# CarbonMatrixLab/AbX

Hardware: AMD Instinct MI355X
Metric: diffusion-steps/sec (100 samples, ~350-res complex) (higher is better)
Workload: dtype f32; 1 GPU; L352: L=352 (Lab 228 + antigen 124), 100 samples of one complex over 1 GPU(s), 1 step = ScoreNetwork (3 passes) + get_prev + reverse, seeded random weights, ESM off; L=352, samples_total=100, chunk=auto, parallelism=sample-shard x1, no collective in the step

## Files before the change

### abx_amd/csrc/gemm_as.hip

```cpp
#include <stdlib.h>

#include <type_traits>

#include "common.h"
#include "abx_hip.h"

namespace {

typedef __attribute__((address_space(3))) void* lds_ptr_t;
typedef const __attribute__((address_space(1))) void* glb_ptr_t;

constexpr int AS_BM = 64, AS_BN = 128, AS_NK = 12, AS_RING = 3;
constexpr int AS_KT = 4096;
constexpr int AS_A = AS_NK * AS_KT;
constexpr int AS_STAGE = 2 * AS_BN * 32;
constexpr int AS_HALF = AS_KT / 2;
constexpr int AS_OFF_RING = AS_A;
constexpr int AS_OFF_ST = AS_OFF_RING + AS_RING * AS_STAGE;
constexpr int AS_OFF_CONST = AS_OFF_ST + 4 * 64 * 4;
constexpr int AS_LDS = AS_OFF_CONST + 2 * 1024;

__device__ __forceinline__ void as_glds16(const void* src, char* dst_wave_base) {
    __builtin_amdgcn_global_load_lds((glb_ptr_t)src, (lds_ptr_t)dst_wave_base, 16, 0, 0);
}
__device__ __forceinline__ unsigned as_vgpr32(unsigned o) {
    asm volatile("" : "+v"(o));
    return o;
}
template <int I> using IC = std::integral_constant<int, I>;
template <int I0, int I1, class F> __device__ __forceinline__ void as_static_for(F&& f) {
    if constexpr (I0 < I1) {
        f(IC<I0>{});
        as_static_for<I0 + 1, I1>(f);
    }
}

template <int ROWS> __device__ __forceinline__ int as_plane_off(int plane, int row, int half) {
    return plane * (ROWS * 32) + row * 32 + ((half ^ ((row >> 3) & 1)) << 4);
}

__device__ __forceinline__ long long as_a_row(const AbxGemm& g, int gri) {
    long long gr = gri;
    if (g.a_pair) {
        int pi, pj;
        if (g.c_split_tile) {
            pair_tile_decode(gri, g.pair_Lp, pi, pj);
            pi = min(pi, g.pair_L - 1);
            pj = min(pj, g.pair_L - 1);
        } else {
            pi = gri / g.pair_Lp;
            pj = min(gri - pi * g.pair_Lp, g.pair_L - 1);
        }
        gr = g.a_pair_transpose > 0 ? (long long)pj * g.pair_L + pi : (long long)pi * g.pair_L + pj;
    } else if (g.a_pair_transpose > 0) {
        const int qi = gri / g.a_pair_transpose;
        gr = (long long)(gri - qi * g.a_pair_transpose) * g.a_pair_transpose + qi;
    }
    return gr;
}

__device__ __forceinline__ void as_issue_a(const AbxGemm& g, char* lds, int m0, int b, int wm) {
    const int lane = threadIdx.x & 63;
    const bool remap = g.a_pair_transpose > 0 || g.a_pair != 0;
    const long long row0 = remap ? 0 : m0;
    const char* baseA = reinterpret_cast<const char*>(g.A + (long long)b * g.sAb + row0 * g.sAm);
    unsigned offA[2];
#pragma unroll
    for (int i = 0; i < 2; ++i) {
        const int r = 16 * i + (lane >> 2), p = lane & 3;
        const int kq = p ^ ((r >> 2) & 3);
        const long long gr = as_a_row(g, min(m0 + wm * 32 + r, g.M - 1));
        offA[i] = (unsigned)(((gr - row0) * g.sAm + kq * 4) * 4);
    }
    char* dst = lds + wm * AS_HALF;
#pragma unroll
    for (int kt = 0; kt < AS_NK; ++kt)
#pragma unroll
        for (int i = 0; i < 2; ++i) as_glds16(baseA + kt * 64 + as_vgpr32(offA[i]), dst + kt * AS_KT + i * 1024);
}

struct AsConv {
    float lshift, m2048;
    f32x2 ls2, lq2;
    int rd0, rd1, wr;
    bool ln, relu;
};
__device__ __forceinline__ void as_conv_init(AsConv& c, const AbxGemm& g) {
    const int lane = threadIdx.x & 63, r = lane & 31, h = lane >> 5, x = (r >> 2) & 3;
    c.rd0 = r * 64 + (((2 * h) ^ x) << 4);
    c.rd1 = r * 64 + (((2 * h + 1) ^ x) << 4);
    c.wr = as_plane_off<32>(0, r, h);
    c.lshift = 0.f;
    c.ls2 = c.lq2 = (f32x2){0.f, 0.f};
    c.m2048 = -2048.0f;
    asm volatile("" : "+v"(c.m2048));
    c.ln = g.ln_csum != nullptr;
    c.relu = g.a_relu != 0;
}
template <bool FIRST>
__device__ __forceinline__ void as_conv_ktile(AsConv& c, char* img) {
    const int lane = threadIdx.x & 63;
    const f32x4 lo = *reinterpret_cast<const f32x4*>(img + c.rd0);
    const f32x4 hi = *reinterpret_cast<const f32x4*>(img + c.rd1);
    float xv[8];
#pragma unroll
    for (int e = 0; e < 4; ++e) { xv[e] = lo[e]; xv[4 + e] = hi[e]; }
    if (c.ln) {
        if (FIRST) c.lshift = __shfl(xv[0], lane & 31, 64);
        const f32x2 sh2 = {c.lshift, c.lshift};
#pragma unroll
        for (int e = 0; e < 4; ++e) {
            f32x2 xp = {xv[2 * e], xv[2 * e + 1]};
            xp -= sh2;
            c.ls2 += xp;
            c.lq2 = __builtin_elementwise_fma(xp, xp, c.lq2);
            xv[2 * e] = xp[0];
            xv[2 * e + 1] = xp[1];
        }
    }
    if (c.relu) {
#pragma unroll
        for (int e = 0; e < 8; ++e) xv[e] = fmaxf(xv[e], 0.f);
    }
    unsigned q0[4], q1[4];
#pragma unroll
    for (int e = 0; e < 4; ++e) split2h_mix(xv[2 * e], xv[2 * e + 1], c.m2048, q0[e], q1[e]);
    *reinterpret_cast<u32x4*>(img + c.wr) = u32x4{q0[0], q0[1], q0[2], q0[3]};
    *reinterpret_cast<u32x4*>(img + c.wr + 1024) = u32x4{q1[0], q1[1], q1[2], q1[3]};
}
__device__ __forceinline__ void as_conv_finish(const AsConv& c, float* st, int wm, float eps, float cs) {
    const int lane = threadIdx.x & 63;
    const float ls = c.ls2[0] + c.ls2[1], lq = c.lq2[0] + c.lq2[1];
    const float invK = 1.0f / (float)(AS_NK * 16);
    const float sm = ls + __shfl_xor(ls, 32, 64), sq = lq + __shfl_xor(lq, 32, 64);
    if (lane < 32) {
        const float dm = sm * invK;
        st[wm * 32 + lane] = dm;
        st[64 + wm * 32 + lane] = (1.0f / sqrtf(fmaxf(sq * invK - dm * dm, 0.f) + eps)) * cs;
    }
}

__device__ __forceinline__ void as_quad_transpose(const float (&x)[4], float (&o)[4]) {
    float a0, a1, a2, a3;
    asm volatile(
        "s_nop 1\n\t"
        "s_mov_b32 vcc_lo, 0x55555555\n\ts_mov_b32 vcc_hi, 0x55555555\n\t"
        "v_cndmask_b32_dpp %4, %9, %8, vcc quad_perm:[1,0,3,2] row_mask:0xf bank_mask:0xf\n\t"
        "v_cndmask_b32_dpp %6, %11, %10, vcc quad_perm:[1,0,3,2] row_mask:0xf bank_mask:0xf\n\t"
        "s_mov_b32 vcc_lo, 0xaaaaaaaa\n\ts_mov_b32 vcc_hi, 0xaaaaaaaa\n\t"
        "v_cndmask_b32_dpp %5, %8, %9, vcc quad_perm:[1,0,3,2] row_mask:0xf bank_mask:0xf\n\t"
        "v_cndmask_b32_dpp %7, %10, %11, vcc quad_perm:[1,0,3,2] row_mask:0xf bank_mask:0xf\n\t"
        "s_mov_b32 vcc_lo, 0x33333333\n\ts_mov_b32 vcc_hi, 0x33333333\n\t"
        "v_cndmask_b32_dpp %0, %6, %4, vcc quad_perm:[2,3,0,1] row_mask:0xf bank_mask:0xf\n\t"
        "v_cndmask_b32_dpp %1, %7, %5, vcc quad_perm:[2,3,0,1] row_mask:0xf bank_mask:0xf\n\t"
        "s_mov_b32 vcc_lo, 0xcccccccc\n\ts_mov_b32 vcc_hi, 0xcccccccc\n\t"
        "v_cndmask_b32_dpp %2, %4, %6, vcc quad_perm:[2,3,0,1] row_mask:0xf bank_mask:0xf\n\t"
        "v_cndmask_b32_dpp %3, %5, %7, vcc quad_perm:[2,3,0,1] row_mask:0xf bank_mask:0xf"
        : "=&v"(o[0]), "=&v"(o[1]), "=&v"(o[2]), "=&v"(o[3]), "=&v"(a0), "=&v"(a1), "=&v"(a2), "=&v"(a3)
        : "v"(x[0]), "v"(x[1]), "v"(x[2]), "v"(x[3])
        : "vcc");
}

template <int S0, int NSL, int NST, int NDMA = 4>
struct AsSched {
    static_assert(S0 >= 2 && S0 + NSL <= 10, "slice window");
    static constexpr int after(int kt, bool first) { return (kt == 0 ? 2 : 0) + ((!first && kt >= S0 && kt < S0 + NSL) ? NST : 0); }
    static constexpr int allow(int kt, bool first) {
        const int k2 = (kt + AS_NK - 2) % AS_NK, k1 = (kt + AS_NK - 1) % AS_NK;
        return after(k2, first) + NDMA + after(k1, first);
    }
};

enum { AS_EPI_PLAIN = 0, AS_EPI_GLU = 1 };

template <int N>
__device__ __forceinline__ void as_rendezvous(u32x4 (&fa)[2], u32x4 (&fb)[2][2]) {
    asm volatile("s_waitcnt vmcnt(%6) lgkmcnt(0)\n\ts_barrier"
                 : "+v"(fa[0]), "+v"(fa[1]), "+v"(fb[0][0]), "+v"(fb[0][1]), "+v"(fb[1][0]), "+v"(fb[1][1])
                 : "n"(N)
                 : "memory");
}
__device__ __forceinline__ void as_rendezvous_free(u32x4 (&fa)[2], u32x4 (&fb)[2][2]) {
    asm volatile("s_waitcnt lgkmcnt(0)\n\ts_barrier"
                 : "+v"(fa[0]), "+v"(fa[1]), "+v"(fb[0][0]), "+v"(fb[0][1]), "+v"(fb[1][0]), "+v"(fb[1][1])
                 :
                 : "memory");
}
template <int N> __device__ __forceinline__ void as_wait_vm() { asm volatile("s_waitcnt vmcnt(%0)" ::"n"(N) : "memory"); }

template <int EPI, bool SIDE, bool EDGE, int ABL = 0, bool PL = false>
__device__ __forceinline__ void as_block(const AbxGemm& g, const AbxGemm& s2, char* lds, int mt, int b) {
    const int lane = threadIdx.x & 63, wave = __builtin_amdgcn_readfirstlane(threadIdx.x >> 6);
    const int wm = wave >> 1, wn = wave & 1, h = lane >> 5;
    const int m0 = mt * AS_BM;
    float* st = reinterpret_cast<float*>(lds + AS_OFF_ST);
    using Sched = typename std::conditional<EPI == AS_EPI_PLAIN, AsSched<2, 8, (ABL == 1 ? 0 : (PL ? 2 : 1)), (ABL == 3 ? 2 : 4)>, AsSched<6, 2, (ABL == 1 ? 0 : 2), (ABL == 3 ? 2 : 4)>>::type;

    const int ntiles = (g.N + AS_BN - 1) / AS_BN;
    const bool ragged = (g.N % AS_BN) != 0;
    const char* bbase = reinterpret_cast<const char*>(g.B_split);
    const long long bkstep = g.sB3k * 2;
    unsigned off0, offU[2];
    {
        const int row = lane >> 1, hp = lane & 1;
        off0 = (unsigned)((wm * g.sB3p + (long long)row * g.sB3n + 8 * (hp ^ ((row >> 3) & 1))) * 2);
#pragma unroll
        for (int i = 2; i < 4; ++i) {
            const int r2 = i * 32 + row;
            const int half = hp ^ ((row >> 3) & 1);
            if (SIDE) offU[i - 2] = (unsigned)((wm * s2.sB3p + (long long)min(r2 - 64, s2.N - 1) * s2.sB3n + 8 * half) * 2);
            else offU[i - 2] = (unsigned)((wm * g.sB3p + (long long)min((ntiles - 1) * AS_BN + r2, g.N - 1) * g.sB3n + 8 * half) * 2);
        }
    }
    const char* bbaseS = SIDE ? reinterpret_cast<const char*>(s2.B_split) : bbase;
    const long long bkstepS = SIDE ? s2.sB3k * 2 : bkstep;
    const unsigned tile_step = (unsigned)(AS_BN * g.sB3n * 2), chunk_step = (unsigned)(32 * g.sB3n * 2);
    auto issue_b = [&](int tile, int kt, int slot, bool half_only = false) __attribute__((always_inline)) {
        char* dst = lds + AS_OFF_RING + slot * AS_STAGE + wm * 4096;
        const int t = min(tile, ntiles - 1);
        const char* src = bbase + kt * bkstep + (long long)t * tile_step;
#pragma unroll
        for (int i = 0; i < 2; ++i) as_glds16(src + i * chunk_step + as_vgpr32(off0), dst + i * 1024);
        if (half_only) return;
        if (t == ntiles - 1) {
            const char* srcU = bbaseS + kt * bkstepS;
#pragma unroll
            for (int i = 2; i < 4; ++i) as_glds16(srcU + as_vgpr32(offU[i - 2]), dst + i * 1024);
        } else {
#pragma unroll
            for (int i = 2; i < 4; ++i) as_glds16(src + i * chunk_step + as_vgpr32(off0), dst + i * 1024);
        }
    };
    const float* csrc = (wm ? g.bias : g.ln_csum);
    auto issue_consts = [&](int tile) __attribute__((always_inline)) {
        const int t = min(tile, ntiles - 1);
#pragma unroll
        for (int i = 0; i < 2; ++i) {
            const int n = min(t * AS_BN + i * 64 + lane, g.N - 1);
            char* dst = lds + AS_OFF_CONST + (tile & 1) * 1024 + wm * 512 + i * 256;
            __builtin_amdgcn_global_load_lds((glb_ptr_t)(csrc + n), (lds_ptr_t)dst, 4, 0, 0);
        }
    };

#ifdef ABX_AS_STAMP
    unsigned long long t_wait = 0, t_vm = 0, t_bar = 0;
    const unsigned long long t_begin = __builtin_amdgcn_s_memtime();
    unsigned long long t_issued = 0, as_t_landed = 0;
#endif
    AsConv cv;
    char* a_half = lds + wm * AS_HALF;
    if (wn == 0) {
        as_issue_a(g, lds, m0, b, wm);
#ifdef ABX_AS_STAMP
        t_issued = __builtin_amdgcn_s_memtime();
#endif
        as_conv_init(cv, g);
        as_wait_vm<20>();
#ifdef ABX_AS_STAMP
        as_t_landed = __builtin_amdgcn_s_memtime();
#endif
        as_conv_ktile<true>(cv, a_half);
        as_conv_ktile<false>(cv, a_half + AS_KT);
    } else {
        issue_b(0, 0, 0);
        issue_b(0, 1, 1);
        issue_b(0, 2, 2);
        if (EPI == AS_EPI_GLU && wm == 0) {
            const int m = m0 + lane;
            int pi, pj;
            pair_tile_decode(m, g.pair_Lp, pi, pj);
            const bool ok = m < g.M && pi < g.pair_L && pj < g.c_split_L;
            st[128 + lane] = (ok && g.rowscale) ? g.rowscale[(long long)b * g.sRSb + (long long)pi * g.pair_Lp + pj] : (ok ? 1.f : 0.f);
            st[192 + lane] = ok ? 1.f : 0.f;
        }
        as_wait_vm<8>();
    }
    __syncthreads();

    const float cs = __builtin_ldexpf(1.0f, -ABX_F16_A_EXP - g.b_exp), inv_cs = __builtin_ldexpf(1.0f, ABX_F16_A_EXP + g.b_exp);
    const float csS = SIDE ? __builtin_ldexpf(1.0f, -ABX_F16_A_EXP - s2.b_exp) : 0.f;
    float* Cb = g.C + (long long)b * g.sCb;
    bool bad = false;

    const int offAf = wm * AS_HALF + as_plane_off<32>(0, lane & 31, h);
    const int offBf = AS_OFF_RING + as_plane_off<AS_BN>(0, wn * 64 + (lane & 31), h);
    u32x4 fa[2][2], fb[2][2][2];
// ... 134 lines not shown
                    for (int c = 0; c < 4; ++c) {
                        const long long mc = mg + c;
                        if (mc < g.M) {
                            const long long sbc = mc / LLs;
                            s2.C[sbc * s2.sCb + (long long)n * s2.sCm + (mc - sbc * LLs)] = v[c];
                        }
                    }
                }
            }
        }
    };

#if defined(ABX_AS_STAMP) && ABX_AS_STAMP >= 2
#define AS_STAMP_PRE unsigned long long ts0_ = __builtin_amdgcn_s_memtime();
#define AS_STAMP_POST t_wait += __builtin_amdgcn_s_memtime() - ts0_;
#else
#define AS_STAMP_PRE
#define AS_STAMP_POST
#endif
    auto step = [&](int tile, auto kt_, auto first_, auto role_) __attribute__((always_inline)) {
        constexpr int kt = decltype(kt_)::value;
        constexpr bool first = decltype(first_)::value != 0;
        constexpr int role = decltype(role_)::value;
        constexpr int set = kt & 1;
        AS_STAMP_PRE
#if defined(ABX_AS_STAMP) && ABX_AS_STAMP >= 3
        if constexpr (role == 1 && !EDGE) {
            const unsigned long long ta_ = __builtin_amdgcn_s_memtime();
            asm volatile("s_waitcnt vmcnt(%6) lgkmcnt(0)"
                         : "+v"(fa[set][0]), "+v"(fa[set][1]), "+v"(fb[set][0][0]), "+v"(fb[set][0][1]), "+v"(fb[set][1][0]), "+v"(fb[set][1][1])
                         : "n"(Sched::allow(kt, first)) : "memory");
            const unsigned long long tb_ = __builtin_amdgcn_s_memtime();
            asm volatile("s_barrier" ::: "memory");
            t_vm += tb_ - ta_;
            t_bar += __builtin_amdgcn_s_memtime() - tb_;
        } else
#endif
        if constexpr (role == 0) as_rendezvous_free(fa[set], fb[set]);
        else if constexpr (EDGE) as_rendezvous<0>(fa[set], fb[set]);
        else as_rendezvous<Sched::allow(kt, first)>(fa[set], fb[set]);
        AS_STAMP_POST
        if constexpr (role == 1) {
            {
                constexpr int k3 = (kt + 3) % AS_NK;
                issue_b(kt + 3 >= AS_NK ? tile + 1 : tile, k3, kt % 3, ABL == 3);
            }
            if constexpr (kt == 0) issue_consts(tile);
        } else if constexpr (first && kt < AS_NK - 2) {
            as_wait_vm<2 * (AS_NK - 3 - kt)>();
            as_conv_ktile<false>(cv, a_half + (kt + 2) * AS_KT);
            if constexpr (kt == AS_NK - 3) as_conv_finish(cv, st, wm, g.ln_eps, cs);
        }
        if constexpr (kt == 1 && !first) read_consts();
        read_frags((kt + 1) & 1, (kt + 1) % AS_NK, (kt + 1) % 3);
        if (ABL == 2) {
#pragma unroll
            for (int j = 0; j < 2; ++j)
#pragma unroll
                for (int e = 0; e < 4; ++e) acc[j][e] = __builtin_bit_cast(float, fa[set][0][e] ^ fb[set][j][0][e] ^ fb[set][j][1][e] ^ fa[set][1][e]);
        } else {
            u32x4 p2[2];
#pragma unroll
            for (int j = 0; j < 2; ++j) p2[j] = f16x8_lo(fb[set][j][0]);
            if constexpr (kt == 0) {
                const f32x16 z = {0.f, 0.f, 0.f, 0.f, 0.f, 0.f, 0.f, 0.f, 0.f, 0.f, 0.f, 0.f, 0.f, 0.f, 0.f, 0.f};
#pragma unroll
                for (int j = 0; j < 2; ++j) acc[j] = mfma_split(fa[set][1], p2[j], z);
            } else {
#pragma unroll
                for (int j = 0; j < 2; ++j) acc[j] = mfma_split(fa[set][1], p2[j], acc[j]);
            }
#pragma unroll
            for (int j = 0; j < 2; ++j) acc[j] = mfma_split(fa[set][0], fb[set][j][1], acc[j]);
#pragma unroll
            for (int j = 0; j < 2; ++j) acc[j] = mfma_split(fa[set][0], fb[set][j][0], acc[j]);
        }
        if constexpr (!first) {
            if constexpr (EPI == AS_EPI_PLAIN) {
                if constexpr (kt >= 2 && kt < 10) plain_slice(IC<kt - 2>{});
            } else {
                if constexpr (kt >= 2 && kt < 6) glu_value(IC<kt - 2>{});
                if constexpr (kt >= 6 && kt < 8) glu_round(IC<kt - 6>{});
            }
        }
    };
    auto rotate = [&](int tile) __attribute__((always_inline)) {
#pragma unroll
        for (int j = 0; j < 2; ++j) accp[j] = acc[j];
        tile_p = tile;
    };

#ifdef ABX_AS_STAMP
    const unsigned long long t_walk0 = __builtin_amdgcn_s_memtime();
    unsigned long long t_walk1 = 0;
#endif
    read_frags(0, 0, 0);
    auto walk = [&](auto role_) __attribute__((always_inline)) {
        as_static_for<0, AS_NK>([&](auto kt_) { step(0, kt_, IC<1>{}, role_); });
        rotate(0);
        for (int tile = 1; tile < ntiles; ++tile) {
            as_static_for<0, AS_NK>([&](auto kt_) { step(tile, kt_, IC<0>{}, role_); });
            rotate(tile);
        }
#ifdef ABX_AS_STAMP
        t_walk1 = __builtin_amdgcn_s_memtime();
#endif
        asm volatile("s_waitcnt vmcnt(0)" ::: "memory");
        constexpr int role = decltype(role_)::value;
        if (SIDE && role == 1) side_store();
        else if (SIDE || !ragged || role == 0) {
            read_consts();
            if constexpr (EPI == AS_EPI_PLAIN) as_static_for<0, 8>([&](auto q_) { plain_slice(q_); });
            else {
                as_static_for<0, 4>([&](auto q_) { glu_value(q_); });
                as_static_for<0, 2>([&](auto q_) { glu_round(q_); });
            }
        }
    };
    if (wn == 0) walk(IC<0>{});
    else walk(IC<1>{});
    if (g.range_flag && __any(bad) && lane == 0) atomicOr(g.range_flag, g.range_tag);
#ifdef ABX_AS_STAMP
    if (g.clock_probe && threadIdx.x == 0) {
        asm volatile("s_waitcnt vmcnt(0)" ::: "memory");
        const unsigned long long t_end = __builtin_amdgcn_s_memtime();
        unsigned long long* rec = g.clock_probe + 16 + (size_t)blockIdx.x * 8;
        rec[0] = t_wait; rec[1] = t_walk1 - t_walk0; rec[2] = t_walk0 - t_begin; rec[3] = t_end - t_walk1;
        rec[4] = t_issued - t_begin; rec[5] = as_t_landed - t_issued; rec[6] = t_end - t_begin; rec[7] = 1ull;
    }
    if (g.clock_probe && threadIdx.x == 64) {
        unsigned long long* rec = g.clock_probe + 16 + ((size_t)gridDim.x + blockIdx.x) * 8;
        rec[0] = t_vm; rec[1] = t_bar; rec[7] = 1ull;
    }
#endif
}

template <int EPI, bool SIDE, int ABL = 0, bool PL = false>
__global__ __launch_bounds__(256, 2) void gemm_as_kernel(const AbxGemm g, const AbxGemm s2) {
    extern __shared__ __attribute__((aligned(16))) float as_smem[];
    char* lds = reinterpret_cast<char*>(as_smem);
    const ClockProbe probe(g.clock_probe);
    const unsigned ntm = (unsigned)((g.M + AS_BM - 1) / AS_BM);
    const unsigned nwg = gridDim.x, bid = blockIdx.x;
    const unsigned q = nwg >> 3, r = nwg & 7, xcd = bid & 7, loc = bid >> 3;
    const unsigned wgid = (xcd < r ? xcd * (q + 1) : r * (q + 1) + (xcd - r) * q) + loc;
    const int b = (int)(wgid / ntm), mt = (int)(wgid - (unsigned)b * ntm);
    bool edge = (mt + 1) * AS_BM > g.M;
    if (EPI == AS_EPI_GLU) edge = edge || (g.pair_L & 7) != 0 || (g.c_split_L & 15) != 0;
    if (edge) as_block<EPI, SIDE, true, ABL, PL>(g, s2, lds, mt, b);
    else as_block<EPI, SIDE, false, ABL, PL>(g, s2, lds, mt, b);
    probe.finish();
}

}

int abx_gemm_as_dispatch(const AbxGemm& g, const AbxGemm* side, hipStream_t st, int* rc) {
    auto al16 = [](const void* p) { return (reinterpret_cast<uintptr_t>(p) & 15) == 0; };
    static const bool off = getenv("ABX_NO_GEMM_AS") != nullptr;
    if (off || (g.tune & 2048)) return 1;
    if (g.exact == 1 || !g.B_split || !g.b_f16 || g.A_split || !g.A || g.sAk != 1 || g.K != AS_NK * 16) return 1;
    if (g.A2 || g.out_ln_w || g.mlp || g.ln_stats || g.gate || g.resid || g.batch_inner || !g.ln_csum || !g.bias) return 1;
    if (g.act != 0 || g.alpha != 1.0f) return 1;
    if (!al16(g.A) || g.sAm % 4 != 0 || g.sAb % 4 != 0 || !al16(g.B_split) || g.sB3n % 8 != 0 || g.sB3p % 8 != 0 || g.sB3k % 8 != 0) return 1;
    if (g.b_exp < -100 || g.b_exp > 100) return 1;
    if (((g.a_pair_transpose > 0 || g.a_pair) ? (long long)g.M * g.sAm : 64LL * g.sAm) >= (1LL << 30)) return 1;
    if ((long long)(g.K / 16) * g.sB3k >= (1LL << 31)) return 1;
    const long long ntm = ((long long)g.M + AS_BM - 1) / AS_BM;
    if (ntm * g.batch >= (1LL << 31)) return 1;
    if (g.N < 256 || ntm * g.batch < 1024) return 1;
    const bool glu = g.glu != 0;
    if (glu) {
        if (side || !g.C_split || !g.c_split_tile || !g.c_transposed || g.N % 128 != 0 || !g.a_pair || g.pair_Lp <= 0 || g.c_split_L != g.pair_Lp || g.c_split_nA % 32 != 0) return 1;
        if (!g.c_vec_ok || (reinterpret_cast<uintptr_t>(g.C_split) & 15) != 0 || g.sCb % 8 != 0 || g.sCm % 8 != 0 || g.sCk % 8 != 0 || g.sCp % 8 != 0) return 1;
        if (g.sB3b != 0) return 1;
    } else {
        if (g.c_transposed || g.C_split || g.rowscale || g.a_pair_transpose > 0 || g.pair_Lp != 0 || g.batch != 1) return 1;
        if (!g.c_vec_ok || g.N % 64 != 0) return 1;
        if (g.c_planes_from > 0 && (!side || g.c_planes_group != 48 || g.c_planes_from % 32 != 0 || (g.N - g.c_planes_from) % 48 != 0 || g.N >= (1 << 16))) return 1;
        if (side) {
            const AbxGemm& s = *side;
            if (g.N % 128 != 64) return 1;
            if (!s.B_split || !s.b_f16 || s.A_split || s.A != g.A || s.sAk != 1 || s.K != g.K || s.sAm != g.sAm || !s.c_transposed || s.N > 32 ||
                s.exact == 1 || (long long)s.M * s.batch != (long long)g.M || (s.batch > 1 && s.sAb != (long long)s.M * s.sAm) ||
                (s.ln_csum == nullptr) != (g.ln_csum == nullptr) || s.ln_stats || s.gate || s.resid || s.rowscale || s.act != 0 || s.glu || s.C_split ||
                s.A2 || s.out_ln_w || s.mlp || s.a_pair_transpose > 0 || s.pair_Lp != 0 || s.a_relu != g.a_relu ||
                !al16(s.B_split) || s.sB3n % 8 != 0 || s.sB3p % 8 != 0 || s.sB3k % 8 != 0 || s.b_exp < -100 || s.b_exp > 100 ||
                (long long)(s.K / 16) * s.sB3k >= (1LL << 31) || (g.ln_csum && s.ln_eps != g.ln_eps))
                return 1;
        }
    }
    static const AbxGemm none = {};
    const dim3 grid((unsigned)(ntm * g.batch)), block(256);
#define AS_LAUNCH(EPI, SIDE, ABL, ...)                                                                                                   \
    do {                                                                                                                                 \
        if (int e = abx_ensure_dynamic_lds(reinterpret_cast<const void*>(&gemm_as_kernel<EPI, SIDE, ABL, ##__VA_ARGS__>), AS_LDS, "abx_gemm(as)")) { \
            *rc = e;                                                                                                                     \
            return 0;                                                                                                                    \
        }                                                                                                                                \
        hipLaunchKernelGGL((gemm_as_kernel<EPI, SIDE, ABL, ##__VA_ARGS__>), grid, block, AS_LDS, st, g, side ? *side : none);            \
    } while (0)
#ifdef ABX_AS_ABLATE
    const int abl = (g.tune >> 12) & 3;
    if (abl == 1) { if (glu) AS_LAUNCH(AS_EPI_GLU, false, 1); else if (side) AS_LAUNCH(AS_EPI_PLAIN, true, 1); else AS_LAUNCH(AS_EPI_PLAIN, false, 1); }
    else if (abl == 2) { if (glu) AS_LAUNCH(AS_EPI_GLU, false, 2); else if (side) AS_LAUNCH(AS_EPI_PLAIN, true, 2); else AS_LAUNCH(AS_EPI_PLAIN, false, 2); }
    else if (abl == 3) { if (glu) AS_LAUNCH(AS_EPI_GLU, false, 3); else if (side) AS_LAUNCH(AS_EPI_PLAIN, true, 3); else AS_LAUNCH(AS_EPI_PLAIN, false, 3); }
    else
#endif
    if (glu) AS_LAUNCH(AS_EPI_GLU, false, 0);
    else if (side && g.c_planes_from > 0) AS_LAUNCH(AS_EPI_PLAIN, true, 0, true);
    else if (side) AS_LAUNCH(AS_EPI_PLAIN, true, 0);
    else AS_LAUNCH(AS_EPI_PLAIN, false, 0);
#undef AS_LAUNCH
    *rc = abx_check_launch("abx_gemm(as)");
    return 0;
}
```

### abx_amd/ops.py

```python
import ctypes as C
import math

import torch

from abx_amd import _lib
from abx_amd._lib import (AbxGemm, AbxTriAttn, AbxIpaTail, AbxHeadsTail, AbxScoreArgs, AbxReverseArgs, AbxGuidanceArgs, AbxDesignScoreArgs, AbxRelaxArgs, AbxInterfaceArgs, AbxEnsemblePairsArgs, AbxEnsembleClusterArgs, AbxLinearPack, AbxLinearSrc,
                           AbxTriMulPack, AbxTriAttnPack, AbxTriRowPack, check)


def _stream():
    return C.c_void_p(torch.cuda.current_stream().cuda_stream)


def _p(t):
    if t is None:
        return None
    assert t.is_cuda, 'libabx_hip works on device memory only'
    return t.data_ptr()


def _f32(t):
    assert t.dtype == torch.float32, t.dtype
    return t


GEMM_TUNE = int(__import__('os').environ.get('ABX_GEMM_TUNE', '0'))

RANGE_TAGS = {'gemm': 1, 'contraction': 2, 'plane_projection': 4, 'tri_mul_tail': 8, 'pair_transition': 16, 'ipa_pair_init': 32,
              'tri_attn': 64, 'ipa_tail': 128, 'heads_tail': 256, 'gemm_late': 512}
RANGE_CHECK = not bool(__import__('os').environ.get('ABX_NO_RANGE_CHECK'))
_range_words = {}


RANGE_SLOTS = 4
RANGE_SLOT = 0


def range_words(device):
    idx = torch.device(device).index
    idx = torch.cuda.current_device() if idx is None else idx
    w = _range_words.get(idx)
    if w is None:
        w = torch.zeros(RANGE_SLOTS, dtype=torch.int32, device=torch.device('cuda', idx))
        _range_words[idx] = w
    return w


def range_word(device):
    return range_words(device)[0:1]


def range_ptr(device):
    return range_words(device).data_ptr() + 4 * RANGE_SLOT


def range_names(bits):
    return [n for n, b in RANGE_TAGS.items() if bits & b]


RANGE_ORDER = ('gemm', 'plane_projection', 'contraction', 'tri_mul_tail', 'tri_attn', 'pair_transition', 'ipa_pair_init', 'gemm_late', 'ipa_tail', 'heads_tail')


def first_range_tag(bits, skip=0):
    for n in RANGE_ORDER:
        if bits & RANGE_TAGS[n] & ~skip:
            return RANGE_TAGS[n]
    return 0


GEMM_EXACT = False


def gemm_kernel_name(M, N, K, batch, a_kcontig=True, b_ncontig=True, transposed=False, split=False, exact=None, a_split=False, dual=False, out_ln=False):
    b = lambda x: 'true' if x else 'false'
    if dual:
        return 'gemm3_dual_kernel<128, 96, 32, 96, 3>'
    if out_ln:
        return 'gemm3_oln_kernel<128, 128, 32, 128, 4>'
    exact = 1 if GEMM_EXACT else int(exact or 0)
    blocks128 = ((M + 127) // 128) * ((N + 127) // 128) * batch
    wide192 = ((N + 191) // 192) * 192 <= ((N + 127) // 128) * 128
    if exact != 1 and split and N <= 32 and a_kcontig and not a_split and K % 16 == 0:
        return f'gemm3_kernel<128, 32, 32, 32, 0, {b(transposed)}, 6>'
    if exact != 1 and split and N > 64 and (blocks128 >= 256 or exact == 2) and K % 16 == 0 and (a_kcontig or a_split or M % 4 == 0):
        amode = 2 if a_split else (0 if a_kcontig else 1)
        pad128, pad192 = ((N + 127) // 128) * 128, ((N + 191) // 192) * 192
        wide = pad192 <= pad128 if a_split else (wide192 and N % 128 != 0)
        cfg = (128, 192, 32, 192, 3) if wide else (128, 128, 32, 128, 4)
        if not wide and blocks128 < 384 and M > 64:
            cfg = (64, 128, 32, 64, 4)
        return f'gemm3_kernel<{cfg[0]}, {cfg[1]}, {cfg[2]}, {cfg[3]}, {amode}, {b(transposed)}, {cfg[4]}>'
    if N <= 32:
        cfg = (128, 32, 32, 32, 3)
    elif N <= 64:
        cfg = (128, 64, 32, 64, 3)
    elif blocks128 < 512:
        cfg = (64, 64, 32, 32, 3)
    elif wide192:
        cfg = (128, 192, 64, 96, 2)
    else:
        cfg = (128, 128, 64, 64, 3)
    return f'gemm_kernel<{cfg[0]}, {cfg[1]}, {cfg[2]}, {cfg[3]}, 16, {b(a_kcontig)}, {b(b_ncontig)}, {b(transposed)}, {cfg[4]}>'


def gemm_as_kernel_name(g, side=None):
    if GEMM_EXACT or (g.tune & 2048) or g.exact == 1 or not g.B_split or not g.b_f16 or g.A_split or not g.A or g.sAk != 1 or g.K != 192:
        return None
    if g.A2 or g.out_ln_w or g.mlp or g.ln_stats or g.gate or g.resid or g.batch_inner or not g.ln_csum or not g.bias or g.act != 0 or g.alpha != 1.0:
        return None
    ntm = (g.M + 63) // 64
    if g.N < 256 or ntm * g.batch < 1024:
        return None
    if g.glu:
        if side is not None or not g.C_split or not g.c_split_tile or not g.c_transposed or g.N % 128 != 0 or not g.a_pair or g.pair_Lp <= 0:
            return None
        return 'gemm_as_kernel<1, false, 0, false>'
    if g.c_transposed or g.C_split or g.rowscale or g.a_pair_transpose > 0 or g.pair_Lp != 0 or g.batch != 1 or g.N % 64 != 0:
        return None
    if side is not None:
        s2 = side
        if g.N % 128 != 64 or not s2.B_split or not s2.c_transposed or s2.N > 32 or s2.K != g.K or s2.M * s2.batch != g.M or s2.act != 0 or s2.exact == 1:
            return None
        return 'gemm_as_kernel<0, true, 0, true>' if g.c_planes_from > 0 else 'gemm_as_kernel<0, true, 0, false>'
    return 'gemm_as_kernel<0, false, 0, false>'


SPLIT_MIN_L = 64


def gemm_mode(L):
    return 1 if (GEMM_EXACT or L < SPLIT_MIN_L) else 2


def gemm_split_eligible(M, N, K, batch=1):
    return (not GEMM_EXACT) and N > 64 and K % 16 == 0 and ((M + 127) // 128) * ((N + 127) // 128) * batch >= 256


def pack_glu_weights(Wv, Wg, bv=None, bg=None):
    K, C_ = Wv.shape
    assert Wg.shape == (K, C_) and C_ % 64 == 0
    W = torch.stack([Wv.reshape(K, C_ // 32, 32), Wg.reshape(K, C_ // 32, 32)], dim=2).reshape(K, 2 * C_).contiguous()
    b = None
    if bv is not None or bg is not None:
        z = torch.zeros(C_, device=Wv.device, dtype=Wv.dtype)
        b = torch.stack([(bv if bv is not None else z).reshape(C_ // 32, 32), (bg if bg is not None else z).reshape(C_ // 32, 32)],
                        dim=1).reshape(2 * C_).contiguous()
    return W, b


_PERM16 = (0, 1, 2, 3, 8, 9, 10, 11, 4, 5, 6, 7, 12, 13, 14, 15)


def permute_k16(Wt):
    K, N = Wt.shape
    assert K % 16 == 0
    idx = torch.tensor(_PERM16, device=Wt.device)
    return Wt.reshape(K // 16, 16, N)[:, idx, :].reshape(K, N).contiguous()


class WeightPlanes(torch.Tensor):
    w_exp = 0
    __torch_function__ = torch._C._disabled_torch_function_impl


def split_weights(Wt):
    K, N = Wt.shape
    _f32(Wt)
    Kp = (K + 15) // 16 * 16
    amax = float(Wt.abs().max())
    if not math.isfinite(amax):
        raise ValueError('split_weights: non-finite weight')
    w_exp = 14 - math.frexp(amax)[1] if amax > 0 else 0
    w_exp = max(-100, min(100, w_exp))
    out = torch.empty(Kp // 16, 2, N, 16, device=Wt.device, dtype=torch.float16)
    check(_lib.load().abx_split_weights_f16(_p(Wt), Wt.stride(1), Wt.stride(0), N, K, w_exp, _p(out), _stream()), 'abx_split_weights_f16')
    out = out.as_subclass(WeightPlanes)
    out.w_exp = w_exp
    return out


def weights_to_float(w3):
    v = (w3[:, 0].float() + w3[:, 1].float()) * 2.0 ** (-w3.w_exp)
    return v.permute(0, 2, 1).reshape(-1, w3.shape[2])


def _weight_planes(w3, N, K=None, what='B3'):
    assert isinstance(w3, WeightPlanes) and w3.dtype == torch.float16 and w3.is_contiguous() and w3.shape[1:] == (2, N, 16), \
        f'{what}: WeightPlanes (ops.split_weights) of N = {N} expected'
    assert K is None or w3.shape[0] * 16 >= K
    return w3


def gemm(A, B, Cout, *, ln=None, a_relu=False, bias=None, alpha=1.0, act=0, rowscale=None, gate=None, gate_sigmoid=True,
         resid=None, tune=None, B3=None, exact=None, a_pair_transpose=0, glu=False, pair=None, a_pair=False, c_pair=False, dual=None, out_ln=None, clock_probe=None, mlp=None, c_split_nA=0, c_split_tile=False,
         defer=False, range_class=None, c_plane_cols=None):
    lib = _lib.load()
    g = AbxGemm()
    a_planes, b_planes, c_planes = A.dtype == torch.int16, B.dtype == torch.int16, Cout.dtype == torch.int16
    if a_planes and A.dim() == 6:
        assert B.dtype == torch.int16 and B.dim() == 6 and B.shape[:2] == A.shape[:2]
        g.batch_inner, g.sA3i, g.sB3i = A.shape[1], A.stride(1), B.stride(1)
        bo_a, bo_b = A.stride(0), B.stride(0)
        A = A.as_strided((A.shape[0] * A.shape[1],) + tuple(A.shape[2:]), (0,) + tuple(A.stride()[2:]), A.storage_offset())
        B = B.as_strided((B.shape[0] * B.shape[1],) + tuple(B.shape[2:]), (0,) + tuple(B.stride()[2:]), B.storage_offset())
    else:
        bo_a = bo_b = None
    if a_planes:
        assert A.dim() == 5 and A.shape[2] == 2 and A.shape[4] == 16 and A.stride(4) == 1
        nb, KT, _, M, _ = A.shape
        K = KT * 16
        g.A_split, g.sA3b, g.sA3k, g.sA3p, g.sA3m = _p(A), (A.stride(0) if nb > 1 else 0), A.stride(1), A.stride(2), A.stride(3)
        if bo_a is not None:
            g.sA3b = bo_a
    else:
        if A.dim() == 2:
            A = A.unsqueeze(0)
        nb, M, K = A.shape
        _f32(A)
        g.A, g.sAb, g.sAm, g.sAk = _p(A), A.stride(0) if nb > 1 else 0, A.stride(1), A.stride(2)
        if a_pair:
            assert pair is not None and M == pair[0] * pair[0], (A.shape, pair)
            M = pair[0] * pair[1]
            if c_split_tile:
                M = ((pair[0] + 7) // 8 * 8) * ((pair[1] + 15) // 16 * 16)
    if b_planes:
        assert B.dim() == 5 and B.shape[2] == 2 and B.shape[4] == 16 and B.stride(4) == 1 and B.shape[1] * 16 == K and B.shape[0] == nb
        N = B.shape[3]
        g.B_split, g.sB3b, g.sB3k, g.sB3p, g.sB3n = _p(B), (B.stride(0) if nb > 1 else 0), B.stride(1), B.stride(2), B.stride(3)
# ... 905 lines not shown
```

Baseline: 168.3 sample-steps/s.

## Add fused dual-GEMM kernel with LN-gate, sigmoid and residual epilogue

Adds a specialized kernel for the dual GEMM case (N=192, K=128 plus a K2=192 gate GEMM). It async-loads both activation tiles and weights into LDS, applies LayerNorm statistics on the fly, and computes the sigmoid gate and residual add in the epilogue. Waves are split by role: some convert and normalise activations while others stream weights. This replaces the generic gemm3_dual_kernel for large batches and is meant to cut memory traffic and kernel overhead. The cost is a lot of new hand-scheduled wait/barrier code with tight eligibility checks.

```diff
diff --git a/abx_amd/csrc/gemm_as.hip b/abx_amd/csrc/gemm_as.hip
--- a/abx_amd/csrc/gemm_as.hip
+++ b/abx_amd/csrc/gemm_as.hip
@@ -98,13 +98,8 @@
     c.relu = g.a_relu != 0;
 }
 template <bool FIRST>
-__device__ __forceinline__ void as_conv_ktile(AsConv& c, char* img) {
+__device__ __forceinline__ void as_conv_values(AsConv& c, float (&xv)[8], char* img) {
     const int lane = threadIdx.x & 63;
-    const f32x4 lo = *reinterpret_cast<const f32x4*>(img + c.rd0);
-    const f32x4 hi = *reinterpret_cast<const f32x4*>(img + c.rd1);
-    float xv[8];
-#pragma unroll
-    for (int e = 0; e < 4; ++e) { xv[e] = lo[e]; xv[4 + e] = hi[e]; }
     if (c.ln) {
         if (FIRST) c.lshift = __shfl(xv[0], lane & 31, 64);
         const f32x2 sh2 = {c.lshift, c.lshift};
@@ -128,10 +123,18 @@
     *reinterpret_cast<u32x4*>(img + c.wr) = u32x4{q0[0], q0[1], q0[2], q0[3]};
     *reinterpret_cast<u32x4*>(img + c.wr + 1024) = u32x4{q1[0], q1[1], q1[2], q1[3]};
 }
-__device__ __forceinline__ void as_conv_finish(const AsConv& c, float* st, int wm, float eps, float cs) {
+template <bool FIRST>
+__device__ __forceinline__ void as_conv_ktile(AsConv& c, char* img) {
+    const f32x4 lo = *reinterpret_cast<const f32x4*>(img + c.rd0);
+    const f32x4 hi = *reinterpret_cast<const f32x4*>(img + c.rd1);
+    float xv[8];
+#pragma unroll
+    for (int e = 0; e < 4; ++e) { xv[e] = lo[e]; xv[4 + e] = hi[e]; }
+    as_conv_values<FIRST>(c, xv, img);
+}
+__device__ __forceinline__ void as_conv_finish(const AsConv& c, float* st, int wm, float eps, float cs, float invK = 1.0f / (float)(AS_NK * 16)) {
     const int lane = threadIdx.x & 63;
     const float ls = c.ls2[0] + c.ls2[1], lq = c.lq2[0] + c.lq2[1];
-    const float invK = 1.0f / (float)(AS_NK * 16);
     const float sm = ls + __shfl_xor(ls, 32, 64), sq = lq + __shfl_xor(lq, 32, 64);
     if (lane < 32) {
         const float dm = sm * invK;
@@ -572,12 +575,357 @@
     probe.finish();
 }
 
+
+constexpr int AD_BN = 192, AD_NK2 = 12, AD_NK1 = 8, AD_NS = AD_NK2 + AD_NK1;
+constexpr int AD_PLANE = AD_BN * 32;
+constexpr int AD_STAGE = 2 * AD_PLANE;
+constexpr int AD_OFF_RING = AS_A;
+constexpr int AD_OFF_ST = AD_OFF_RING + 2 * AD_STAGE;
+constexpr int AD_OFF_CONST = AD_OFF_ST + 4 * 64 * 4;
+constexpr int AD_LDS = AD_OFF_CONST + 4 * AD_BN * 4;
+static_assert(AD_LDS <= 81920, "two blocks per CU");
+constexpr int AD_P0 = 4;
+constexpr int ad_wslot(int t) { return t < 4 ? AD_OFF_RING + (t & 1) * AD_STAGE : ((t - 4) % 3 == 0 ? AD_OFF_RING : ((t - 4) % 3 == 1 ? 0 : AD_OFF_RING + AD_STAGE)); }
+
+__device__ __forceinline__ void ad_issue_z(const AbxGemm& g, char* lds, int m0, int b, int wm) {
+    const int lane = threadIdx.x & 63;
+    const bool remap = g.pair_Lp > 0;
+    const long long row0 = remap ? 0 : m0;
+    const char* baseA = reinterpret_cast<const char*>(g.A2 + (long long)b * g.sA2b + row0 * g.sA2m);
+    unsigned offA[2];
+#pragma unroll
+    for (int i = 0; i < 2; ++i) {
+        const int r = 16 * i + (lane >> 2), p = lane & 3;
+        const int kq = p ^ ((r >> 2) & 3);
+        const int gri = min(m0 + wm * 32 + r, g.M - 1);
+        long long gr = gri;
+        if (remap) {
+            const int pi = gri / g.pair_Lp, pj = min(gri - pi * g.pair_Lp, g.pair_L - 1);
+            gr = (long long)pi * g.pair_L + pj;
+        }
+        offA[i] = (unsigned)(((gr - row0) * g.sA2m + kq * 4) * 4);
+    }
+    char* dst = lds + wm * AS_HALF;
+#pragma unroll
+    for (int kt = 0; kt < AD_NK2; ++kt)
+#pragma unroll
+        for (int i = 0; i < 2; ++i) as_glds16(baseA + kt * 64 + as_vgpr32(offA[i]), dst + kt * AS_KT + i * 1024);
+}
+
+template <bool FIRST>
+__device__ __forceinline__ void ad_conv_ptile(AsConv& c, char* img) {
+    const int lane = threadIdx.x & 63, r = lane & 31, h = lane >> 5;
+    float xv[8];
+#pragma unroll
+    for (int e = 0; e < 8; ++e) xv[e] = *reinterpret_cast<const float*>(img + (8 * h + e) * 128 + r * 4);
+    as_conv_values<FIRST>(c, xv, img);
+}
+
+__device__ __forceinline__ void ad_rendezvous(u32x4 (&fa)[2], u32x4 (&fb)[3][2]) {
+    asm volatile("s_waitcnt lgkmcnt(0)\n\ts_barrier"
+                 : "+v"(fa[0]), "+v"(fa[1]), "+v"(fb[0][0]), "+v"(fb[0][1]), "+v"(fb[1][0]), "+v"(fb[1][1]), "+v"(fb[2][0]), "+v"(fb[2][1])
+                 :
+                 : "memory");
+}
+template <int N>
+__device__ __forceinline__ void ad_rendezvous_vm(u32x4 (&fa)[2], u32x4 (&fb)[3][2]) {
+    asm volatile("s_waitcnt vmcnt(%8) lgkmcnt(0)\n\ts_barrier"
+                 : "+v"(fa[0]), "+v"(fa[1]), "+v"(fb[0][0]), "+v"(fb[0][1]), "+v"(fb[1][0]), "+v"(fb[1][1]), "+v"(fb[2][0]), "+v"(fb[2][1])
+                 : "n"(N)
+                 : "memory");
+}
+
+template <bool EDGE>
+__device__ __forceinline__ void as_dual_block(const AbxGemm& g, char* lds, int mt, int b) {
+    const int lane = threadIdx.x & 63, wave = __builtin_amdgcn_readfirstlane(threadIdx.x >> 6);
+    const int wm = wave >> 1, wn = wave & 1, h = lane >> 5;
+    const int m0 = mt * AS_BM;
+    float* st = reinterpret_cast<float*>(lds + AD_OFF_ST);
+    const float* cc = reinterpret_cast<const float*>(lds + AD_OFF_CONST);
+
+    const char* wbase2 = reinterpret_cast<const char*>(g.B2_split);
+    const char* wbase1 = reinterpret_cast<const char*>(g.B_split + (long long)b * g.sB3b);
+    const long long wk2 = g.sB23k * 2, wk1 = g.sB3k * 2;
+    const unsigned wchunk2 = (unsigned)(32 * g.sB23n * 2), wchunk1 = (unsigned)(32 * g.sB3n * 2);
+    unsigned woff2, woff1;
+    {
+        const int row = lane >> 1, half = (lane & 1) ^ ((row >> 3) & 1);
+        woff2 = (unsigned)((wm * g.sB23p + (long long)row * g.sB23n + 8 * half) * 2);
+        woff1 = (unsigned)((wm * g.sB3p + (long long)row * g.sB3n + 8 * half) * 2);
+    }
+    auto issue_w = [&](auto s_) __attribute__((always_inline)) {
+        constexpr int s = decltype(s_)::value;
+        char* dst = lds + ad_wslot(s) + wm * AD_PLANE;
+        if constexpr (s < AD_NK2) {
+            const char* src = wbase2 + s * wk2;
+#pragma unroll
+            for (int i = 0; i < 6; ++i) as_glds16(src + i * wchunk2 + as_vgpr32(woff2), dst + i * 1024);
+        } else {
+            const char* src = wbase1 + (s - AD_NK2) * wk1;
+#pragma unroll
+            for (int i = 0; i < 6; ++i) as_glds16(src + i * wchunk1 + as_vgpr32(woff1), dst + i * 1024);
+        }
+    };
+
+    const char* pbase = reinterpret_cast<const char*>(g.A + (long long)b * g.sAb + m0);
+    const long long pk = 16LL * g.sAk * 4;
+    unsigned poff[2];
+#pragma unroll
+    for (int i = 0; i < 2; ++i) {
+        const int kl = 8 * i + (lane >> 3);
+        const int gm = min(m0 + wm * 32 + 4 * (lane & 7), g.M - 4) - m0;
+        poff[i] = (unsigned)(((long long)kl * g.sAk + gm) * 4);
+    }
+    auto issue_p = [&](int kt) __attribute__((always_inline)) {
+        char* dst = lds + (AD_P0 + kt) * AS_KT + wm * AS_HALF;
+        const char* src = pbase + kt * pk;
+#pragma unroll
+        for (int i = 0; i < 2; ++i) as_glds16(src + as_vgpr32(poff[i]), dst + i * 1024);
+    };
+
+    const float cs2 = __builtin_ldexpf(1.0f, -ABX_F16_A_EXP - g.b2_exp), inv_cs2 = __builtin_ldexpf(1.0f, ABX_F16_A_EXP + g.b2_exp);
+    const float cs1 = __builtin_ldexpf(1.0f, -ABX_F16_A_EXP - g.b_exp), inv_cs1 = __builtin_ldexpf(1.0f, ABX_F16_A_EXP + g.b_exp);
+    AsConv cz, cp;
+    char* a_half = lds + wm * AS_HALF;
+    if (wn == 0) {
+        ad_issue_z(g, lds, m0, b, wm);
+        as_conv_init(cz, g);
+        cz.ln = true;
+        cz.relu = false;
+        cp = cz;
+        as_wait_vm<20>();
+        as_conv_ktile<true>(cz, a_half);
+        as_conv_ktile<false>(cz, a_half + AS_KT);
+    } else {
+        const float* c0 = wm ? g.ln_csum : g.ln2_csum;
+        const float* c1 = wm ? g.bias : g.bias2;
+#pragma unroll
+        for (int a = 0; a < 2; ++a)
+#pragma unroll
+            for (int i = 0; i < 3; ++i) {
+                char* dst = lds + AD_OFF_CONST + (2 * wm + a) * (AD_BN * 4) + i * 256;
+                __builtin_amdgcn_global_load_lds((glb_ptr_t)((a ? c1 : c0) + i * 64 + lane), (lds_ptr_t)dst, 4, 0, 0);
+            }
+        issue_w(IC<0>{});
+        issue_w(IC<1>{});
+        as_wait_vm<6>();
+    }
+    __syncthreads();
+
+    const int offAf = wm * AS_HALF + as_plane_off<32>(0, lane & 31, h);
+    const int offBf = as_plane_off<AD_BN>(0, wn * 96 + (lane & 31), h);
+    u32x4 fa[2][2], fb[2][3][2];
+    auto read_frags = [&](int set, int kt, int wslot) __attribute__((always_inline)) {
+#pragma unroll
+        for (int p = 0; p < 2; ++p) fa[set][p] = *reinterpret_cast<const u32x4*>(lds + kt * AS_KT + offAf + p * 1024);
+#pragma unroll
+        for (int j = 0; j < 3; ++j)
+#pragma unroll
+            for (int p = 0; p < 2; ++p) fb[set][j][p] = *reinterpret_cast<const u32x4*>(lds + offBf + wslot + p * AD_PLANE + j * 1024);
+    };
+
+    f32x16 gatev[3], acc[3];
+    const float* st_w = st + wm * 32 + 4 * h;
+    auto gate_values = [&]() __attribute__((always_inline)) {
+#pragma unroll
+        for (int j = 0; j < 3; ++j) {
+            const int n = wn * 96 + j * 32 + (lane & 31);
+            const float csum2 = cc[n] * inv_cs2, bias2 = cc[AD_BN + n];
+#pragma unroll
+            for (int rq = 0; rq < 4; ++rq) {
+                const f32x4 dm4 = *reinterpret_cast<const f32x4*>(st_w + 8 * rq), rs4 = *reinterpret_cast<const f32x4*>(st_w + 64 + 8 * rq);
+#pragma unroll
+                for (int c = 0; c < 4; ++c) {
+                    const float gv = rs4[c] * (gatev[j][4 * rq + c] - dm4[c] * csum2) + bias2;
+                    gatev[j][4 * rq + c] = sigmoidf_(gv);
+                }
+            }
+        }
+    };
+
+    f32x4 rv[4][3];
+    long long row_off_c[4];
+    bool row_ok[4];
+    auto load_resid = [&]() __attribute__((always_inline)) {
+        const float* rd = g.resid + (long long)b * g.sRb;
+#pragma unroll
+        for (int rq = 0; rq < 4; ++rq) {
+            const int m = m0 + wm * 32 + 8 * rq + 4 * h + (lane & 3);
+            bool ok = !EDGE || m < g.M;
+            long long mo = m;
+            if (g.c_pair) {
+                const int pi = m / g.pair_Lp, pj = m - pi * g.pair_Lp;
+                ok = ok && pj < g.pair_L;
+                mo = (long long)pi * g.pair_L + pj;
+            }
+            row_ok[rq] = ok;
+            row_off_c[rq] = mo * g.sCm;
+#pragma unroll
+            for (int j = 0; j < 3; ++j) {
+                const int n = wn * 96 + j * 32 + ((lane & 31) >> 2) * 4;
+                rv[rq][j] = (f32x4){0.f, 0.f, 0.f, 0.f};
+                if (ok) rv[rq][j] = *reinterpret_cast<const f32x4*>(rd + mo * g.sRm + n);
+            }
+        }
+    };
+
+    auto step = [&](auto s_, auto role_) __attribute__((always_inline)) {
+        constexpr int s = decltype(s_)::value, role = decltype(role_)::value, set = s & 1;
+        if constexpr (role == 0) ad_rendezvous(fa[set], fb[set]);
+        else ad_rendezvous_vm<(s >= 3 && s + 2 < AD_NS) ? 6 : 0>(fa[set], fb[set]);
+        if constexpr (role == 1) {
+            if constexpr (s < 2) issue_w(IC<s + 2>{});
+            else if constexpr (s == 2) { issue_w(IC<4>{}); issue_w(IC<5>{}); }
+            else if constexpr (s + 3 < AD_NS) issue_w(IC<s + 3>{});
+        } else {
+            constexpr int np = s < AD_P0 ? 0 : (s - AD_P0 + 1 < AD_NK1 ? s - AD_P0 + 1 : AD_NK1);
+            if constexpr (s >= AD_P0 && s < AD_P0 + AD_NK1) issue_p(s - AD_P0);
+            if constexpr (s < AD_NK2 - 2) {
+                as_wait_vm<(24 - 2 * (s + 3)) + 2 * np>();
+                as_conv_ktile<false>(cz, a_half + (s + 2) * AS_KT);
+                if constexpr (s == AD_NK2 - 3) as_conv_finish(cz, st, wm, g.ln_eps, cs2);
+            } else if constexpr (s < AD_NK2) {
+                as_wait_vm<2 * (np - 1 - (s - 10))>();
+                ad_conv_ptile<s == 10>(cp, a_half + (AD_P0 + s - 10) * AS_KT);
+            } else if constexpr (s - AD_NK2 + 2 < AD_NK1) {
+                constexpr int kp = s - AD_NK2 + 2;
+                as_wait_vm<2 * (AD_NK1 - 1 - kp)>();
+                ad_conv_ptile<false>(cp, a_half + (AD_P0 + kp) * AS_KT);
+                if constexpr (kp == AD_NK1 - 1) as_conv_finish(cp, st + 128, wm, g.ln_eps, cs1, 1.0f / (float)(AD_NK1 * 16));
+            }
+        }
+        if constexpr (s + 1 < AD_NS) read_frags((s + 1) & 1, (s + 1) < AD_NK2 ? s + 1 : s + 1 - AD_NK2 + AD_P0, ad_wslot(s + 1));
+        u32x4 p2[3];
+#pragma unroll
+        for (int j = 0; j < 3; ++j) p2[j] = f16x8_lo(fb[set][j][0]);
+        if constexpr (s < AD_NK2) {
+            if constexpr (s == 0) {
+                const f32x16 z = {0.f, 0.f, 0.f, 0.f, 0.f, 0.f, 0.f, 0.f, 0.f, 0.f, 0.f, 0.f, 0.f, 0.f, 0.f, 0.f};
+#pragma unroll
+                for (int j = 0; j < 3; ++j) gatev[j] = mfma_split(fa[set][1], p2[j], z);
+            } else {
+#pragma unroll
+                for (int j = 0; j < 3; ++j) gatev[j] = mfma_split(fa[set][1], p2[j], gatev[j]);
+            }
+#pragma unroll
+            for (int j = 0; j < 3; ++j) gatev[j] = mfma_split(fa[set][0], fb[set][j][1], gatev[j]);
+#pragma unroll
+            for (int j = 0; j < 3; ++j) gatev[j] = mfma_split(fa[set][0], fb[set][j][0], gatev[j]);
+        } else {
+            if constexpr (s == AD_NK2) {
+                const f32x16 z = {0.f, 0.f, 0.f, 0.f, 0.f, 0.f, 0.f, 0.f, 0.f, 0.f, 0.f, 0.f, 0.f, 0.f, 0.f, 0.f};
+#pragma unroll
+                for (int j = 0; j < 3; ++j) acc[j] = mfma_split(fa[set][1], p2[j], z);
+            } else {
+#pragma unroll
+                for (int j = 0; j < 3; ++j) acc[j] = mfma_split(fa[set][1], p2[j], acc[j]);
+            }
+#pragma unroll
+            for (int j = 0; j < 3; ++j) acc[j] = mfma_split(fa[set][0], fb[set][j][1], acc[j]);
+#pragma unroll
+            for (int j = 0; j < 3; ++j) acc[j] = mfma_split(fa[set][0], fb[set][j][0], acc[j]);
+        }
+        if constexpr (s == AD_NK2) gate_values();
+    };
+
+    read_frags(0, 0, ad_wslot(0));
+    auto walk = [&](auto role_) __attribute__((always_inline)) { as_static_for<0, AD_NS>([&](auto s_) { step(s_, role_); }); };
+    if (wn == 0) walk(IC<0>{});
+    else walk(IC<1>{});
+
+    float* Cb = g.C + (long long)b * g.sCb;
+    bool bad = false;
+    load_resid();
+#pragma unroll
+    for (int j = 0; j < 3; ++j) {
+        const int nl = wn * 96 + j * 32 + (lane & 31);
+        const float csum1 = cc[2 * AD_BN + nl] * inv_cs1, bias1 = cc[3 * AD_BN + nl];
+        const int n = wn * 96 + j * 32 + ((lane & 31) >> 2) * 4;
+#pragma unroll
+        for (int rq = 0; rq < 4; ++rq) {
+            const f32x4 dm4 = *reinterpret_cast<const f32x4*>(st_w + 128 + 8 * rq), rs4 = *reinterpret_cast<const f32x4*>(st_w + 192 + 8 * rq);
+            float x[4], o[4];
+#pragma unroll
+            for (int c = 0; c < 4; ++c) {
+                float v = rs4[c] * (acc[j][4 * rq + c] - dm4[c] * csum1);
+                v = v + bias1;
+                x[c] = v * gatev[j][4 * rq + c];
+            }
+            as_quad_transpose(x, o);
+            f32x4 ov;
+#pragma unroll
+            for (int c = 0; c < 4; ++c) {
+                ov[c] = o[c] + rv[rq][j][c];
+                bad |= row_ok[rq] && __builtin_amdgcn_classf(ov[c], 0x207);
+            }
+            if (row_ok[rq]) *reinterpret_cast<f32x4*>(Cb + row_off_c[rq] + n) = ov;
+        }
+    }
+    if (g.range_flag && __any(bad) && lane == 0) atomicOr(g.range_flag, g.range_tag);
+}
+
+__global__ __launch_bounds__(256, 2) void gemm_as_dual_kernel(const AbxGemm g) {
+    extern __shared__ __attribute__((aligned(16))) float as_smem[];
+    char* lds = reinterpret_cast<char*>(as_smem);
+    const ClockProbe probe(g.clock_probe);
+    const unsigned ntm = (unsigned)((g.M + AS_BM - 1) / AS_BM);
+    const unsigned nwg = gridDim.x, bid = blockIdx.x;
+    const unsigned q = nwg >> 3, r = nwg & 7, xcd = bid & 7, loc = bid >> 3;
+    const unsigned wgid = (xcd < r ? xcd * (q + 1) : r * (q + 1) + (xcd - r) * q) + loc;
+    const int b = (int)(wgid / ntm), mt = (int)(wgid - (unsigned)b * ntm);
+    if ((mt + 1) * AS_BM > g.M) as_dual_block<true>(g, lds, mt, b);
+    else as_dual_block<false>(g, lds, mt, b);
+    probe.finish();
+}
+
+int as_dual_dispatch(const AbxGemm& g, hipStream_t st, int* rc) {
+    auto al16 = [](const void* p) { return (reinterpret_cast<uintptr_t>(p) & 15) == 0; };
+    static const bool off = [] {
+        const char* e = getenv("ABX_NO_DUAL_AS");
+        return e != nullptr && !(e[0] == '0' && e[1] == 0);
+    }();
+    if (off) return 1;
+    if (g.exact == 1 || g.K != AD_NK1 * 16 || g.K2 != AD_NK2 * 16 || g.N != AD_BN) return 1;
+    if (!g.A || g.A_split || g.sAm != 1 || g.M % 4 != 0 || g.M < 4 || !g.B_split || !g.B2_split || !g.b_f16) return 1;
+    if (!g.ln_csum || g.ln_stats || !g.ln2_csum || !g.bias || !g.bias2 || !g.resid || !g.C) return 1;
+    if (g.act != 0 || g.alpha != 1.0f || g.gate || g.mlp || g.glu || g.rowscale || g.out_ln_w || g.C_split || g.c_transposed || g.a_relu ||
+        g.a_pair_transpose > 0 || g.a_pair || g.c_split_tile || g.batch_inner || g.c_planes_from)
+        return 1;
+    if (!g.c_vec_ok || !g.r_vec_ok) return 1;
+    const long long rows_c = g.c_pair ? (long long)g.pair_L * g.pair_L : g.M;
+    auto overlaps = [&](const float* p, long long sb, long long sm) {
+        const float* c1 = g.C + (g.batch - 1) * g.sCb + (rows_c - 1) * g.sCm + AD_BN;
+        const float* p1 = p + (g.batch - 1) * sb + (rows_c - 1) * sm + AD_BN;
+        return g.C < p1 && p < c1;
+    };
+    if (overlaps(g.A2, g.sA2b, g.sA2m) || overlaps(g.resid, g.sRb, g.sRm)) return 1;
+    if (!al16(g.A) || g.sAk % 4 != 0 || g.sAb % 4 != 0 || !al16(g.A2) || g.sA2m % 4 != 0 || g.sA2b % 4 != 0) return 1;
+    if (!al16(g.B_split) || g.sB3n % 8 != 0 || g.sB3p % 8 != 0 || g.sB3k % 8 != 0 || g.sB3b % 8 != 0) return 1;
+    if (!al16(g.B2_split) || g.sB23n % 8 != 0 || g.sB23p % 8 != 0 || g.sB23k % 8 != 0) return 1;
+    if (g.b_exp < -100 || g.b_exp > 100 || g.b2_exp < -100 || g.b2_exp > 100) return 1;
+    if ((g.pair_Lp > 0 ? (long long)g.pair_L * g.pair_L * g.sA2m : 64LL * g.sA2m) >= (1LL << 30)) return 1;
+    if (16LL * g.sAk + g.M >= (1LL << 30)) return 1;
+    if (g.sB3p + AD_BN * g.sB3n >= (1LL << 30) || g.sB23p + AD_BN * g.sB23n >= (1LL << 30)) return 1;
+    if ((long long)AD_NK1 * g.sB3k >= (1LL << 31) || (long long)AD_NK2 * g.sB23k >= (1LL << 31)) return 1;
+    const long long ntm = ((long long)g.M + AS_BM - 1) / AS_BM;
+    if (ntm * g.batch >= (1LL << 31)) return 1;
+    if (!(g.tune & 16384) && ntm * g.batch < 1024) return 1;
+    if (int e = abx_ensure_dynamic_lds(reinterpret_cast<const void*>(&gemm_as_dual_kernel), AD_LDS, "abx_gemm(as, dual)")) {
+        *rc = e;
+        return 0;
+    }
+    hipLaunchKernelGGL(gemm_as_dual_kernel, dim3((unsigned)(ntm * g.batch)), dim3(256), AD_LDS, st, g);
+    *rc = abx_check_launch("abx_gemm(as, dual)");
+    return 0;
+}
+
 }
 
 int abx_gemm_as_dispatch(const AbxGemm& g, const AbxGemm* side, hipStream_t st, int* rc) {
     auto al16 = [](const void* p) { return (reinterpret_cast<uintptr_t>(p) & 15) == 0; };
     static const bool off = getenv("ABX_NO_GEMM_AS") != nullptr;
     if (off || (g.tune & 2048)) return 1;
+    if (g.A2) return side ? 1 : as_dual_dispatch(g, st, rc);
     if (g.exact == 1 || !g.B_split || !g.b_f16 || g.A_split || !g.A || g.sAk != 1 || g.K != AS_NK * 16) return 1;
     if (g.A2 || g.out_ln_w || g.mlp || g.ln_stats || g.gate || g.resid || g.batch_inner || !g.ln_csum || !g.bias) return 1;
     if (g.act != 0 || g.alpha != 1.0f) return 1;
diff --git a/abx_amd/ops.py b/abx_amd/ops.py
--- a/abx_amd/ops.py
+++ b/abx_amd/ops.py
@@ -74,6 +74,10 @@
 def gemm_kernel_name(M, N, K, batch, a_kcontig=True, b_ncontig=True, transposed=False, split=False, exact=None, a_split=False, dual=False, out_ln=False):
     b = lambda x: 'true' if x else 'false'
     if dual:
+        tune = GEMM_TUNE or 0
+        if (not GEMM_EXACT and int(exact or 0) != 1 and not (tune & 2048) and N == 192 and K == 128 and not a_kcontig and M % 4 == 0
+                and not transposed and split and (((M + 63) // 64) * batch >= 1024 or (tune & 16384))):
+            return 'gemm_as_dual_kernel'
         return 'gemm3_dual_kernel<128, 96, 32, 96, 3>'
     if out_ln:
         return 'gemm3_oln_kernel<128, 128, 32, 128, 4>'
```

Result: faster. 170.7 sample-steps/s, median of 6 (+1.4%).
